# nschejtman/deepLoopCloser

Hardware: AMD Instinct MI355X
Metric: query-frames/sec vs N-keyframe DB + top-k recall@1 (higher is better)
Workload: dtype bf16; 1 GPU; 1000000 x 4096 bf16 keyframe DB, Q=256, top-20 cosine match, 1 GPU(s); db_rows=1000000, dim=4096, k=20, rows_per_gpu=1000000, pipelined=False, crowded=False

## Files before the change

### deeploopcloser_amd/_lib.py

```python
import ctypes as C
import os

_HERE = os.path.dirname(os.path.abspath(__file__))
LIB_PATH = os.path.join(_HERE, "libdlc_hip.so")

DLC_OK = 0
DLC_ERR_BAD_ARG, DLC_ERR_BAD_SHAPE, DLC_ERR_UNSUPPORTED, DLC_ERR_HIP, DLC_ERR_WORKSPACE = -1, -2, -3, -4, -5
DLC_BF16, DLC_F16, DLC_F32, DLC_F64, DLC_I8, DLC_U8 = 0, 1, 2, 3, 4, 5
DLC_ACT_NONE, DLC_ACT_SIGMOID, DLC_ACT_RELU = 0, 1, 2
DLC_B_KN, DLC_B_NK = 0, 1
DLC_MAX_K = 128
DLC_ABI_VERSION = 12
DLC_SELECT_COOP = 1
DLC_SIM_FORCE_F64, DLC_SIM_NO_HOST_SYNC = 1, 2

_vp, _i64, _int, _sz, _dbl, _flt = C.c_void_p, C.c_int64, C.c_int, C.c_size_t, C.c_double, C.c_float

SIGNATURES = {
    "dlc_abi_version": (_int, []),
    "dlc_create": (_int, [_int, C.POINTER(_vp)]),
    "dlc_destroy": (_int, [_vp]),
    "dlc_last_error": (C.c_char_p, [_vp]),
    "dlc_status_string": (C.c_char_p, [_int]),
    "dlc_gemm_bias_act": (_int, [_vp, _int, _int, _int, _i64, _i64, _i64, _vp, _i64, _vp, _i64, _vp, _vp, _i64, _vp]),
    "dlc_bias_act": (_int, [_vp, _int, _int, _i64, _i64, _vp, _i64, _vp, _vp, _i64, _vp]),
    "dlc_sdav_encode_workspace_bytes": (_sz, [_i64, C.POINTER(_i64), _int, _int]),
    "dlc_sdav_encode": (_int, [_vp, _int, _i64, _int, C.POINTER(_i64), _vp, C.POINTER(_vp), C.POINTER(_vp), _vp, _vp,
                               _sz, _vp]),
    "dlc_sdav_split_panels_bytes": (_sz, [_int, C.POINTER(_i64)]),
    "dlc_sdav_split_prepare": (_int, [_vp, _int, C.POINTER(_i64), C.POINTER(_vp), _vp, _sz, _vp]),
    "dlc_sdav_encode_split_workspace_bytes": (_sz, [_i64, C.POINTER(_i64), _int]),
    "dlc_cnnvtl_split_panels_bytes": (_sz, [_int, C.POINTER(C.c_int32)]),
    "dlc_cnnvtl_split_prepare": (_int, [_vp, _int, C.POINTER(C.c_int32), C.POINTER(_vp), _vp, _sz, _vp]),
    "dlc_cnnvtl_encode_split_workspace_bytes": (_sz, [_i64, _int, _int, _int, _int, C.POINTER(C.c_int32)]),
    "dlc_cnnvtl_encode_split": (_int, [_vp, _int, _vp, _i64, _int, _int, _int, _int, _int, C.POINTER(C.c_int32), _vp, C.POINTER(_vp),
# ... 53 lines not shown
                                    _vp, _sz, _vp]),
    "dlc_cosine_score_error_bound": (_dbl, [_i64, _i64, _i64, _int]),
    "dlc_cosine_score_error_bound_any_plan": (_dbl, [_i64]),
    "dlc_cosine_score_groups": (_int, [_vp, _int, _vp, _i64, _i64, _vp, _i64, _i64, _i64, _int, _vp, _sz, _vp]),
    "dlc_cosine_select_topk": (_int, [_vp, _int, _vp, _i64, _i64, _vp, _i64, _i64, _i64, _int, _i64, _vp, _vp, _vp, _vp, _vp, _vp,
                                     _sz, _int, _vp]),
    "dlc_cosine_groups_per_query": (_int, [_int]),
    "dlc_cosine_select_groups": (_int, [_vp, _int, _vp, _i64, _i64, _vp, _i64, _i64, _i64, _int, _vp, _sz, _vp, _vp, _int,
                                       _vp]),
    "dlc_cosine_rescore_topk": (_int, [_vp, _int, _vp, _i64, _i64, _vp, _i64, _i64, _i64, _int, _i64, _vp, _vp, _vp, _int,
                                      _vp, _vp, _vp, _vp, _int, _vp]),
    "dlc_cosine_exhaustive_topk": (_int, [_vp, _int, _vp, _i64, _i64, _vp, _i64, _i64, _i64, _int, _i64, _vp, _i64, _dbl,
                                         _vp, _vp, _vp, _vp, _vp, _vp, _sz, _vp]),
    "dlc_topk_merge_strided": (_int, [_vp, _vp, _i64, _vp, _i64, _int, _i64, _int, _vp, _dbl, _vp, _vp, _vp, _vp, _vp, _vp]),
    "dlc_topk_merge": (_int, [_vp, _vp, _vp, _int, _i64, _int, _vp, _vp, _vp, _vp]),
    "dlc_topk_keep_older": (_int, [_vp, _vp, _vp, _i64, _int, _i64, _int, _vp, _vp, _vp]),
    "dlc_cosine_scores_workspace_bytes": (_sz, [_i64, _i64, _i64]),
    "dlc_cosine_scores": (_int, [_vp, _int, _vp, _i64, _i64, _vp, _i64, _i64, _i64, _vp, _i64, _vp, _sz, _vp]),
    "dlc_host_to_device": (_int, [_vp, _vp, _vp, _sz, _vp]),
    "dlc_device_to_host": (_int, [_vp, _vp, _vp, _sz, _vp]),
    "dlc_set_host_threads": (_int, [_vp, _int]),
    "dlc_set_scratch": (_int, [_vp, _vp, _sz]),
    "dlc_set_profiling": (_int, [_vp, _int]),
    "dlc_profile_gemm_ms": (_int, [_vp, C.POINTER(_flt), _int]),
}

_lib = None


class DlcError(RuntimeError):
    """A HIP-side failure (DLC_ERR_HIP / DLC_ERR_WORKSPACE) reported by the C ABI."""


def load():
    global _lib
    if _lib is not None:
        return _lib
    if not os.path.exists(LIB_PATH):
        raise ImportError(
            "deeploopcloser_amd: %s is missing -- build it with `python -c 'import __graft_entry__ as g; g.build()'` "
            "or `make -C deeploopcloser_amd/csrc`.  There is no CPU fallback." % LIB_PATH)
    lib = C.CDLL(LIB_PATH)
    for name, (res, args) in SIGNATURES.items():
        fn = getattr(lib, name)
        fn.restype = res
        fn.argtypes = args
# ... 16 lines not shown
```

### deeploopcloser_amd/csrc/api.hip

```cpp
#include "dlc_internal.h"

#include <new>

extern "C" int dlc_abi_version(void) { return DLC_ABI_VERSION; }

extern "C" const char* dlc_status_string(int status) {
    switch (status) {
        case DLC_OK: return "ok";
        case DLC_ERR_BAD_ARG: return "bad argument";
        case DLC_ERR_BAD_SHAPE: return "bad shape";
        case DLC_ERR_UNSUPPORTED: return "unsupported dtype or mode";
        case DLC_ERR_HIP: return "HIP runtime error";
        case DLC_ERR_WORKSPACE: return "workspace too small";
        default: return "unknown status";
    }
}

extern "C" int dlc_create(int device, dlc_ctx** out) {
    if (!out) return DLC_ERR_BAD_ARG;
    *out = nullptr;
    int count = 0;
    if (hipGetDeviceCount(&count) != hipSuccess || count < 1) return DLC_ERR_HIP;
    if (device < 0 || device >= count) return DLC_ERR_BAD_ARG;
    dlc_ctx* c = new (std::nothrow) dlc_ctx;
// ... 46 lines not shown
    delete ctx->host_lock;
    delete ctx;
    return DLC_OK;
}

extern "C" const char* dlc_last_error(const dlc_ctx* ctx) { return ctx ? ctx->err : "null context"; }

extern "C" int dlc_set_scratch(dlc_ctx* ctx, void* scratch, size_t bytes) {
    if (!ctx) return DLC_ERR_BAD_ARG;
    if ((scratch && bytes == 0) || ((uintptr_t)scratch & 255))
        return dlc::fail(ctx, DLC_ERR_BAD_ARG, "set_scratch: need a 256-byte aligned buffer (or NULL, 0)");
    ctx->scratch = scratch;
    ctx->scratch_bytes = scratch ? bytes : 0;
    return DLC_OK;
}

extern "C" int dlc_set_profiling(dlc_ctx* ctx, int enabled) {
    if (!ctx) return DLC_ERR_BAD_ARG;
    ctx->profiling = enabled ? 1 : 0;
    ctx->prof_calls = 0;
    return DLC_OK;
}

extern "C" int dlc_profile_gemm_ms(dlc_ctx* ctx, float* out_ms, int capacity) {
    if (!ctx) return DLC_ERR_BAD_ARG;
    if (!out_ms || capacity < 1) return dlc::fail(ctx, DLC_ERR_BAD_ARG, "profile_gemm_ms: bad output");
    dlc::DeviceGuard guard(ctx->device);
    long long n = ctx->prof_calls;
    if (n > DLC_PROFILE_RING) n = DLC_PROFILE_RING;
    if (n > capacity) n = capacity;
    for (long long i = 0; i < n; ++i) {
        const long long call = ctx->prof_calls - n + i;
        const int slot = (int)(call % DLC_PROFILE_RING);
        DLC_HIP_CHECK(ctx, hipEventSynchronize(ctx->ev_stop[slot]));
        float ms = 0.f;
        DLC_HIP_CHECK(ctx, hipEventElapsedTime(&ms, ctx->ev_start[slot], ctx->ev_stop[slot]));
        out_ms[i] = ms;
    }
    return (int)n;
}
```

### deeploopcloser_amd/csrc/cosine_topk.hip

```cpp
#include "dlc_internal.h"

#include <algorithm>

namespace {

constexpr int BM = 256;
constexpr int BNQ = 256;
constexpr int BK = 64;
constexpr int NTHREADS = 512;
constexpr int TILE_BYTES = 256 * BK * 2;
constexpr int A_TILE = TILE_BYTES;
constexpr int B_TILE = TILE_BYTES;
#ifndef DLC_A_STAGES
#define DLC_A_STAGES 2
#endif
constexpr int A_STAGES = DLC_A_STAGES;
constexpr int B_RING = A_STAGES * A_TILE;
constexpr int LDS_BYTES = A_STAGES * A_TILE + 2 * B_TILE;
#ifndef DLC_STAGGER_SLEEP
#define DLC_STAGGER_SLEEP 15
#endif
#ifndef DLC_STAGGER_PHASES
#define DLC_STAGGER_PHASES 32
#endif
// ... 33 lines not shown
    const char* Q;
    const char* DB;
    long long ldq_b;
    long long lddb_b;
    int q;
    long long n;
    int nk;
    float* gmax;
    long long ldg;
    float* tmax;
    long long ldt;
    long long ng;
    long long nh;
    float* S;
    long long lds;
    int stagger_mult;
    int stagger_phases;
    int nqb;
    long long ntiles;
    int nsplit;
    int kchunk;
    float* P;
    long long ldp;
};

constexpr int GEMM_GROUPS = 0;
constexpr int GEMM_DENSE = 1;
constexpr int GEMM_PARTIAL = 2;

constexpr int HALF_BYTES = 128 * 128;

#ifndef DLC_A_CACHE_POLICY
#define DLC_A_CACHE_POLICY " nt"
#endif
#define DLC_DMA4_BODY(POLICY)                                \
    asm volatile(                                            \
        "s_nop 4\n\t"                                        \
        "s_mov_b32 %0, m0\n\t"                               \
        "s_mov_b32 m0, %6\n\t"                               \
        "s_nop 0\n\t"                                        \
        "global_load_lds_dwordx4 %1, %5" POLICY "\n\t"       \
        "s_add_u32 m0, %6, 0x400\n\t"                        \
        "s_nop 0\n\t"                                        \
        "global_load_lds_dwordx4 %2, %5" POLICY "\n\t"       \
        "s_add_u32 m0, %6, 0x800\n\t"                        \
        "s_nop 0\n\t"                                        \
        "global_load_lds_dwordx4 %3, %5" POLICY "\n\t"       \
// ... 186 lines not shown
        for (int c = 0; c < 4; ++c) {
            const int qidx = qblk * BNQ + wc * 64 + c * 16 + i;
            if (qidx >= p.q) continue;
#pragma unroll
            for (int t = 0; t < 8; ++t) {
                const long long row0 = tile * BM + wr * 128 + (t >> 2) * 64 + 16 * lg + 4 * (t & 3);
                *(f32x4_t*)(part + (long long)qidx * p.ldp + row0) = acc[t][c];
            }
        }
    } else if constexpr (MODE == GEMM_DENSE) {
#pragma unroll
        for (int c = 0; c < 4; ++c) {
            const int qidx = qblk * BNQ + wc * 64 + c * 16 + i;
            if (qidx >= p.q) continue;
#pragma unroll
            for (int t = 0; t < 8; ++t) {
                const long long row0 = tile * BM + wr * 128 + (t >> 2) * 64 + 16 * lg + 4 * (t & 3);
#pragma unroll
                for (int r = 0; r < 4; ++r)
                    if (row0 + r < p.n) p.S[(long long)qidx * p.lds + row0 + r] = acc[t][c][r];
            }
        }
    } else {
#pragma unroll
        for (int c = 0; c < 4; ++c) {
            const int qidx = qblk * BNQ + wc * 64 + c * 16 + i;
            float hm[2];
#pragma unroll
            for (int th = 0; th < 2; ++th) {
                float m0 = acc[th * 4][c][0], m1 = acc[th * 4 + 2][c][0];
#pragma unroll
                for (int tt = 0; tt < 2; ++tt)
#pragma unroll
                    for (int r = 0; r < 4; ++r) {
                        m0 = fmaxf(m0, acc[th * 4 + tt][c][r]);
                        m1 = fmaxf(m1, acc[th * 4 + 2 + tt][c][r]);
                    }
                hm[th] = fmaxf(m0, m1);
                const long long g = tile * (BM / GROUP) + wr * 16 + th * 8 + lg * 2;
                if (qidx < p.q) {
                    float* dst = p.gmax + (long long)qidx * p.ldg + g;
                    if (g + 1 < p.ng) *(float2*)dst = make_float2(m0, m1);
                    else if (g < p.ng) dst[0] = m0;
                }
            }
            float h = fmaxf(hm[0], hm[1]);
            h = fmaxf(h, __shfl_xor(h, 16));
            h = fmaxf(h, __shfl_xor(h, 32));
            const long long ht = tile * 2 + wr;
            if (lg == 0 && qidx < p.q && ht < p.nh) p.tmax[(long long)qidx * p.ldt + ht] = h;
        }
    }
}

template <typename Tag> struct Dot2;
template <> struct Dot2<dlc_bf16_tag> {
    typedef __attribute__((ext_vector_type(2))) __bf16 v2_t;
    static __device__ __forceinline__ float run(unsigned a, unsigned b, float c) {
        return __builtin_amdgcn_fdot2_f32_bf16(__builtin_bit_cast(v2_t, a), __builtin_bit_cast(v2_t, b), c, false);
    }
};
template <> struct Dot2<dlc_f16_tag> {
    typedef __attribute__((ext_vector_type(2))) _Float16 v2_t;
    static __device__ __forceinline__ float run(unsigned a, unsigned b, float c) {
        return __builtin_amdgcn_fdot2(__builtin_bit_cast(v2_t, a), __builtin_bit_cast(v2_t, b), c, false);
    }
};

constexpr int GEMV_MAX_Q = 4;
constexpr int GEMV_MAX_LDS = 64 * 1024;

template <typename Tag, int QB>
__global__ __launch_bounds__(256) void score_gemv_kernel(GemmArgs p) {
// ... 237 lines not shown
    float* tmax; long long ldt; int nh; int tv_in_lds;
    const float* gmax; long long ldg; long long ng;
    int kg;
    const char* Q; long long ldq_b; const char* DB; long long lddb_b;
    long long n; int d; int k; long long row_offset;
    float* out_s;
    double* out_s64;
    long long* out_i;
    int* status;
    double tau;
    const float* tau_scale;
    int* grp_ids;
    float* grp_max;
    const float* all_max;
    int parts;
    long long nq;
    int gparts;
    float* bound_out;
    const float* dense_S;
    long long ld_s;
    int rslack;
    int limited;
    long long limit0;
};
__device__ __forceinline__ long long visible_rows(long long n, int limited, long long limit0, int qi) {
    if (!limited) return n;
    const long long lim = limit0 + qi;
    return lim < 0 ? 0 : (lim < n ? lim : n);
}

template <typename Tag, int THREADS, int RS_UNROLL, int MODE>
__device__ __forceinline__ void finish_topk_body(const FinishArgs& a) {
    extern __shared__ __attribute__((aligned(16))) char dsm[];
    constexpr int FIN_WAVES = THREADS / 64;
    constexpr int FIN_THREADS = THREADS;
    constexpr int GPH = GROUPS_PER_HALF;
    const int kg = a.kg, k = a.k;
    const double tau = scaled_tau(a.tau, a.tau_scale, (int)blockIdx.x);
    const long long n = visible_rows(a.n, a.limited, a.limit0, (int)blockIdx.x);
    const long long ng = a.limited ? (n + GROUP - 1) / GROUP : a.ng;
    if (n <= 0) {
        if constexpr (MODE == FIN_GROUPS) {
            for (int e = threadIdx.x; e <= kg; e += THREADS) {
                if (e < kg) a.grp_ids[(long long)blockIdx.x * kg + e] = -1;
                a.grp_max[(long long)blockIdx.x * (kg + 1) + e] = -INFINITY;
            }
// ... 108 lines not shown
    }
    __syncthreads();
    kg2 = min(kg, m2);
    rank_select(ckey, m2, kg2, sel2, true);
    __syncthreads();
    if (sel2[kg2] >= 0) bkey = max(bkey, (unsigned)(ckey[sel2[kg2]] >> 32));
    if constexpr (MODE == FIN_GROUPS) {
        const long long W = kg + 1;
        for (int e = tid; e < kg; e += FIN_THREADS) {
            const int c = e < kg2 ? sel2[e] : -1;
            a.grp_ids[(long long)qi * kg + e] = c < 0 ? -1 : (int)key_id(ckey[c]);
            a.grp_max[(long long)qi * W + e] = c < 0 ? -INFINITY : a.gmax[(long long)qi * a.ldg + key_id(ckey[c])];
        }
        if (tid == 0) a.grp_max[(long long)qi * W + kg] = bkey ? key_f32(bkey) : -INFINITY;
        return;
    }
    if (tid < kg2) {
        const int c = sel2[tid];
        int g = c < 0 ? -1 : (int)key_id(ckey[c]);
        if (tid >= k && g >= 0 && sel2[k - 1] >= 0 && !(a.limited && !a.dense_S)) {
            const double uk = (double)key_f32((unsigned)(ckey[sel2[k - 1]] >> 32));
            if ((double)key_f32((unsigned)(ckey[c] >> 32)) < uk - 2.0 * tau) g = -2;
        }
        misc[9] = 0u;
        crow[tid] = g;
    }
    __syncthreads();
    if (tid < kg2) {
        const int g = crow[tid];
        if (g == -2) atomicMax(&misc[9], (unsigned)(ckey[sel2[tid]] >> 32));
    }
    __syncthreads();
    if (tid < kg2) sel2[tid] = crow[tid] < 0 ? -1 : crow[tid];
    bkey = max(bkey, misc[9]);
    __syncthreads();
    } else {
        kg2 = kg;
        const long long W = kg + 1;
        if (a.parts > 0) {
            unsigned bk = 0u;
            for (int e = tid; e < a.parts * (int)W; e += FIN_THREADS) {
                const int pp = e / (int)W, j = e % (int)W;
                const float v = a.all_max[((long long)pp * a.nq + qi) * W + j];
                if (v == -INFINITY) continue;
                if (j == kg) { bk = max(bk, f32_key(v)); continue; }
                int greater = 0;
                for (int p2 = 0; p2 < a.parts; ++p2) {
                    const float* av = a.all_max + ((long long)p2 * a.nq + qi) * W;
// ... 6 lines not shown
        for (int e = tid; e < kg; e += FIN_THREADS) {
            int g = a.grp_ids[(long long)qi * kg + e];
            if (g >= 0 && a.parts > 0) {
                const float v = a.grp_max[(long long)qi * W + e];
                int greater = 0;
                for (int pp = 0; pp < a.parts; ++pp) {
                    const float* av = a.all_max + ((long long)pp * a.nq + qi) * W;
                    for (int j = 0; j < kg; ++j) greater += av[j] > v ? 1 : 0;
                }
                if (greater >= kg) g = -1;
            }
            if (a.gparts > 1 && e % a.gparts != (int)blockIdx.y) g = -1;
            sel2[e] = g;
        }
        __syncthreads();
        if (a.parts > 0) bkey = misc[8];
        else {
            const float v = a.grp_max[(long long)qi * W + kg];
            bkey = v == -INFINITY ? 0u : f32_key(v);
        }
        if (a.bound_out && blockIdx.y == 0 && tid == 0) a.bound_out[qi] = bkey ? key_f32(bkey) : -INFINITY;
    }

    int m3;
    if (a.dense_S) {
        const int m = kg2 * GROUP;
        for (int e = tid; e < m; e += FIN_THREADS) {
            const int g = sel2[e / GROUP];
            const long long row = (long long)g * GROUP + (e % GROUP);
            ckey[e] = (g >= 0 && row < n) ? pack_key(a.dense_S[(long long)qi * a.ld_s + row], (unsigned)row) : 0ull;
        }
        m3 = min(k + a.rslack, m);
        for (int e = tid; e <= m3 && e < kg * GROUP; e += FIN_THREADS) crow[e] = -1;
        __syncthreads();
        if (m3 < m) rank_select(ckey, m, m3, crow, true);
        else rank_select(ckey, m, m3, crow, false);
        __syncthreads();
        if (m3 < m && crow[m3] >= 0) bkey = max(bkey, (unsigned)(ckey[crow[m3]] >> 32));
        __syncthreads();
        for (int e = tid; e < m3; e += FIN_THREADS) { const int c = crow[e]; crow[e] = c < 0 ? -1 : (int)key_id(ckey[c]); }
    } else {
        m3 = kg2 * GROUP;
        for (int e = tid; e < m3; e += FIN_THREADS) {
            const int g = sel2[e / GROUP];
            const long long row = (long long)g * GROUP + (e % GROUP);
            crow[e] = (g >= 0 && row < n) ? (int)row : -1;
        }
    }
    __syncthreads();

    const char* qrow = a.Q + (long long)qi * a.ldq_b;
    if (MODE == FIN_FUSED && a.dense_S != nullptr) {
        for (int ci = w; ci < m3; ci += FIN_WAVES) {
            const int id = __builtin_amdgcn_readfirstlane(crow[ci]);
            const double sc = id < 0 ? 0.0 : rescore1_f64<Tag>(qrow, a.DB + (long long)id * a.lddb_b, a.d, lane);
            if (lane == 0) {
                cs64[ci] = id < 0 ? -INFINITY : sc;
                ck64[ci] = id < 0 ? KEY64_EMPTY : f64_key(sc);
            }
        }
    } else
    for (int s = w; s * GROUP < m3; s += FIN_WAVES) {
        int ids[GROUP];
        bool any = false;
        const char* rows[GROUP];
#pragma unroll
        for (int r = 0; r < GROUP; ++r) {
            ids[r] = __builtin_amdgcn_readfirstlane(s * GROUP + r < m3 ? crow[s * GROUP + r] : -1);
            any |= ids[r] >= 0;
            rows[r] = a.DB + (long long)(ids[r] < 0 ? 0 : ids[r]) * a.lddb_b;
        }
        double acc[GROUP] = {0.0, 0.0, 0.0, 0.0, 0.0, 0.0, 0.0, 0.0};
        if (any) rescore8_f64<Tag, RS_UNROLL>(qrow, rows, a.d, lane, acc);
#pragma unroll
        for (int r = 0; r < GROUP; ++r)
            if (lane == r && s * GROUP + r < m3) {
                cs64[s * GROUP + r] = ids[r] < 0 ? -INFINITY : acc[r];
                ck64[s * GROUP + r] = ids[r] < 0 ? KEY64_EMPTY : f64_key(acc[r]);
            }
    }
    const long long oq = (long long)blockIdx.y * a.nq + qi;
    for (int e = tid; e < k; e += FIN_THREADS) {
        if (a.out_s) a.out_s[oq * k + e] = -INFINITY;
        a.out_s64[oq * k + e] = -INFINITY;
        a.out_i[oq * k + e] = -1;
    }
    for (int e = tid; e <= kg; e += FIN_THREADS) sel[e] = -1;
    __syncthreads();

    rank_select64(ck64, crow, m3, k, sel);
    __syncthreads();
    for (int e = tid; e < k; e += FIN_THREADS) {
        const int c = sel[e];
        if (c >= 0) {
            if (a.out_s) a.out_s[oq * k + e] = (float)cs64[c];
            a.out_s64[oq * k + e] = cs64[c];
            a.out_i[oq * k + e] = (long long)crow[c] + a.row_offset;
        }
    }
    if constexpr (MODE == FIN_FUSED) {
        if (tid == 0) {
            const int c = sel[k - 1];
// ... 552 lines not shown
    const int64_t base = dlc::cdiv(ntiles, (int64_t)8) * 8 * dlc::cdiv(q, BNQ);
    const int64_t nk = d / BK;
    SplitPlan best{1, (int)nk};
    if (base >= 256 || nk < 8) return best;
    const double t_k = 1.6, t_fix = 8.0, t_launch = 5.0, bytes_per_us = 3.0e6;
    const double part_bytes = (double)q * (double)ntiles * BM * 4.0;
    const int64_t work = ntiles * dlc::cdiv(q, BNQ);
    double best_t = (double)dlc::cdiv(work, (int64_t)256) * ((double)nk * t_k + t_fix);
    for (int64_t ns = 2; ns <= nk / 4 && ns <= 256; ++ns) {
        const int64_t kc = dlc::cdiv(nk, ns), ns_eff = dlc::cdiv(nk, kc);
        if (ns_eff != ns) continue;
        if ((double)ns_eff * part_bytes > (double)(1ll << 30)) break;
        const double t = (double)dlc::cdiv(work * ns_eff, (int64_t)256) * ((double)kc * t_k + t_fix) +
                         2.0 * (double)ns_eff * part_bytes / bytes_per_us + t_launch;
        if (t < best_t * 0.9) {
            best_t = t;
            best = SplitPlan{(int)ns_eff, (int)kc};
        }
    }
    return best;
}

struct WsLayout {
    size_t gmax, tmax, part, status, s64, rs_ids, rs_max, rs_scores, rs_idx, rs_bound, total;
    long long ldg, ldt, ldp;
    int kg;
    SplitPlan sp;
    int rparts;
    bool dense;
    double tau;
};

inline bool gemv_shape(int64_t q, int64_t nk) {
    const int qb = q <= 1 ? 1 : (q <= 2 ? 2 : 4);
    return q <= GEMV_MAX_Q && (long long)qb * nk * 128 <= GEMV_MAX_LDS;
}

constexpr int64_t DENSE_MAX_ROWS = 16384;
constexpr int DENSE_ROW_SLACK = 4;
constexpr int64_t DENSE_GEMV_BYTES = 32ll << 20;
inline bool dense_plan(int64_t q, int64_t n, int64_t d) {
    return n <= DENSE_MAX_ROWS && (!gemv_shape(q, d / BK) || n * d * 2 <= DENSE_GEMV_BYTES);
}

int rescore_parts(int64_t q, int64_t d, int kg, int k) {
    if (q > 32 || (int64_t)kg * GROUP * d * 2 < (2 << 20)) return 1;
    return std::min(kg, 2048 / k);
}

constexpr double SCORE_STEP_EPS = 1.1920928955078125e-07;
double score_error_bound(int64_t q, int64_t nk, const SplitPlan& sp, bool dense) {
    double steps;
    if (!dense && gemv_shape(q, nk)) steps = (double)nk * 0.5 + 8.0;
    else steps = 2.0 * (double)sp.kchunk + 2.0;
    return SCORE_STEP_EPS * 1.01 * steps + 3.7e-12;
}

WsLayout ws_layout(int64_t q, int64_t n, int64_t d, int k) {
    WsLayout w;
    const int64_t ntiles = dlc::cdiv(n, BM);
    w.ldg = ntiles * (BM / GROUP);
    w.ldt = ntiles * 2;
    w.kg = k + SLACK;
    size_t o = 0;
    w.gmax = o; o += dlc::align_up((size_t)q * w.ldg * 4, 256);
    w.tmax = o; o += dlc::align_up((size_t)q * w.ldt * 4, 256);
    w.sp = split_plan(q, n, d);
    w.dense = dense_plan(q, n, d);
    w.tau = score_error_bound(q, d / BK, w.sp, w.dense);
    w.ldp = ntiles * BM;
    w.part = o;
    if (w.sp.nsplit > 1 || w.dense) o += dlc::align_up((size_t)w.sp.nsplit * q * w.ldp * 4, 256);
    w.status = o; o += dlc::align_up((size_t)q * 4, 256);
    w.s64 = o; o += dlc::align_up((size_t)q * k * 8, 256);
    w.rparts = w.dense ? 1 : rescore_parts(q, d, w.kg, k);
    w.rs_ids = w.rs_max = w.rs_scores = w.rs_idx = w.rs_bound = o;
    if (w.rparts > 1) {
        w.rs_ids = o; o += dlc::align_up((size_t)q * w.kg * 4, 256);
        w.rs_max = o; o += dlc::align_up((size_t)q * (w.kg + 1) * 4, 256);
        w.rs_scores = o; o += dlc::align_up((size_t)w.rparts * q * k * 8, 256);
        w.rs_idx = o; o += dlc::align_up((size_t)w.rparts * q * k * 8, 256);
        w.rs_bound = o; o += dlc::align_up((size_t)q * 4, 256);
    }
    w.total = o;
    return w;
}

int check_operands(dlc_ctx* ctx, int dtype, const void* Q, int64_t q, int64_t ldq, const void* DB, int64_t n,
                   int64_t lddb, int64_t d) {
// ... 111 lines not shown
    WsLayout w;
};

int prepare_match(dlc_ctx* ctx, const char* what, int dtype, const void* Q, int64_t q, int64_t ldq, const void* DB,
                  int64_t n, int64_t lddb, int64_t d, int k, void* workspace, size_t workspace_bytes, MatchCall* mc) {
    int rc = check_operands(ctx, dtype, Q, q, ldq, DB, n, lddb, d);
    if (rc != DLC_OK) return rc;
    if (k < 1 || k > DLC_MAX_K) return dlc::fail(ctx, DLC_ERR_BAD_ARG, "%s: k=%d outside 1..%d", what, k, DLC_MAX_K);
    mc->w = ws_layout(q, n, d, k);
    if (!workspace || workspace_bytes < mc->w.total)
        return dlc::fail(ctx, DLC_ERR_WORKSPACE, "%s: workspace %zu < %zu bytes", what, workspace_bytes, mc->w.total);
    if (((uintptr_t)workspace & 255)) return dlc::fail(ctx, DLC_ERR_BAD_ARG, "%s: workspace must be 256-byte aligned", what);
    char* ws = (char*)workspace;
    GemmArgs& a = mc->a;
    a.Q = (const char*)Q; a.DB = (const char*)DB;
    a.ldq_b = ldq * 2; a.lddb_b = lddb * 2;
    a.q = (int)q; a.n = n; a.nk = (int)(d / BK);
    a.gmax = (float*)(ws + mc->w.gmax); a.ldg = mc->w.ldg;
    a.tmax = (float*)(ws + mc->w.tmax); a.ldt = mc->w.ldt;
    a.ng = dlc::cdiv(n, GROUP); a.nh = dlc::cdiv(n, HALF);
    a.S = nullptr; a.lds = 0;
    a.nsplit = mc->w.sp.nsplit; a.kchunk = mc->w.sp.kchunk;
    a.P = (float*)(ws + mc->w.part); a.ldp = mc->w.ldp;
    return DLC_OK;
}

inline bool small_direct(const MatchCall& mc, int k) {
    return mc.w.dense && mc.a.n <= (int64_t)FIN_THREADS * SMALL_GPT * GROUP && k + DENSE_ROW_SLACK + 1 <= SMALL_KT_MAX;
}

int run_score(dlc_ctx* ctx, int dtype, MatchCall& mc, hipStream_t st, bool partials_only = false) {
    return dlc::profiled(ctx, st, [&]() -> int {
        return (dtype == DLC_BF16) ? launch_scores<dlc_bf16_tag>(ctx, mc.a, false, st, mc.w.dense, partials_only)
                                   : launch_scores<dlc_f16_tag>(ctx, mc.a, false, st, mc.w.dense, partials_only);
    });
}

FinishArgs finish_args(const MatchCall& mc, int k, int64_t n, int64_t d, int64_t q, int64_t row_offset) {
    const GemmArgs& g = mc.a;
    FinishArgs f{};
    f.tmax = g.tmax; f.ldt = g.ldt; f.nh = (int)g.nh;
    f.gmax = g.gmax; f.ldg = g.ldg; f.ng = g.ng;
    f.kg = mc.w.kg;
    f.Q = g.Q; f.ldq_b = g.ldq_b; f.DB = g.DB; f.lddb_b = g.lddb_b;
    f.n = n; f.d = (int)d; f.k = k; f.row_offset = row_offset;
    f.tau = mc.w.tau;
    f.nq = q;
    return f;
}

template <typename Tag, int THREADS, int RS_UNROLL, int MODE>
int launch_finish(dlc_ctx* ctx, FinishArgs f, int64_t q, bool small_lds, hipStream_t st) {
    size_t dsm = fin_lds_fixed(f.kg);
    f.tv_in_lds = MODE != FIN_RESCORE && !small_lds && (size_t)f.nh * 4 <= 96 * 1024;
    if (f.tv_in_lds) dsm += (size_t)f.nh * 4;
    dsm = dlc::align_up(dsm, 16);
    void (*fk)(FinishArgs);
    if constexpr (THREADS == 256) fk = finish_topk_coop_kernel<Tag, RS_UNROLL, MODE>;
    else fk = finish_topk_kernel<Tag, THREADS, RS_UNROLL, MODE>;
    if (dsm > 48 * 1024)
        DLC_HIP_CHECK(ctx, hipFuncSetAttribute((const void*)fk, hipFuncAttributeMaxDynamicSharedMemorySize, (int)dsm));
    hipLaunchKernelGGL(fk, dim3((unsigned)q, (unsigned)(MODE == FIN_RESCORE && f.gparts > 1 ? f.gparts : 1)), dim3(THREADS),
                       dsm, st, f);
    DLC_LAUNCH_CHECK(ctx, "finish_topk_kernel");
    return DLC_OK;
}

template <int MODE>
int run_select(dlc_ctx* ctx, int dtype, const FinishArgs& f, int64_t q, int flags, hipStream_t st) {
    const bool coop = (flags & DLC_SELECT_COOP) != 0;
// ... 21 lines not shown
    DLC_LAUNCH_CHECK(ctx, "exhaustive_topk_kernel");
    return DLC_OK;
}

int launch_merge(dlc_ctx* ctx, const double* scores, int64_t score_part_stride, const int64_t* idx, int64_t idx_part_stride,
                 int parts, int64_t q, int k, const float* bound, double tau, const float* tau_scale, float* out_scores,
                 double* out_scores_f64, int64_t* out_idx, int* status, hipStream_t st) {
    const size_t m = (size_t)parts * k;
    const size_t dsm = m * 24;
    if (dsm > 48 * 1024) return dlc::fail(ctx, DLC_ERR_BAD_SHAPE, "topk_merge: parts*k=%zu too large (max 2048)", m);
    hipLaunchKernelGGL(merge_topk_kernel, dim3((unsigned)q), dim3(FIN_THREADS), dsm, st, scores, (long long)score_part_stride,
                       (const long long*)idx, (long long)idx_part_stride, parts, (long long)q, k, bound, tau, tau_scale,
                       out_scores, out_scores_f64, (long long*)out_idx, status);
    DLC_LAUNCH_CHECK(ctx, "merge_topk_kernel");
    return DLC_OK;
}

int run_finish(dlc_ctx* ctx, int dtype, const MatchCall& mc, int k, int64_t n, int64_t d, int64_t q, int64_t row_offset,
               float* out_scores, double* out_scores_f64, int64_t* out_idx, int32_t* out_status, void* workspace, int flags,
               const float* tau_scale, hipStream_t st, int limited = 0, int64_t limit0 = 0, bool direct = false) {
    char* ws = (char*)workspace;
    FinishArgs f = finish_args(mc, k, n, d, q, row_offset);
    f.limited = limited; f.limit0 = limit0; f.tau_scale = tau_scale;
    int* status = out_status ? out_status : (int*)(ws + mc.w.status);
    double* s64 = out_scores_f64 ? out_scores_f64 : (double*)(ws + mc.w.s64);
    int rc;
    if (direct) {
        SmallArgs sa{};
        sa.P = mc.a.P; sa.ldp = mc.a.ldp; sa.qstride = (long long)q * mc.a.ldp; sa.nsplit = mc.a.nsplit;
        sa.gmax = mc.a.gmax; sa.ldg = mc.a.ldg;
        sa.Q = f.Q; sa.ldq_b = f.ldq_b; sa.DB = f.DB; sa.lddb_b = f.lddb_b;
        sa.n = n; sa.d = (int)d; sa.k = k; sa.m3max = k + DENSE_ROW_SLACK; sa.row_offset = row_offset;
        sa.out_s = out_scores; sa.out_s64 = s64; sa.out_i = (long long*)out_idx; sa.status = status; sa.tau = mc.w.tau;
        sa.tau_scale = tau_scale; sa.limited = limited; sa.limit0 = limit0;
        const bool long_rows = d >= 16384;
        if (dtype == DLC_BF16) {
            if (long_rows) hipLaunchKernelGGL(small_topk_long_kernel<dlc_bf16_tag>, dim3((unsigned)q), dim3(FIN_THREADS), 0, st, sa);
            else hipLaunchKernelGGL(small_topk_kernel<dlc_bf16_tag>, dim3((unsigned)q), dim3(FIN_THREADS), 0, st, sa);
        } else {
            if (long_rows) hipLaunchKernelGGL(small_topk_long_kernel<dlc_f16_tag>, dim3((unsigned)q), dim3(FIN_THREADS), 0, st, sa);
            else hipLaunchKernelGGL(small_topk_kernel<dlc_f16_tag>, dim3((unsigned)q), dim3(FIN_THREADS), 0, st, sa);
        }
        DLC_LAUNCH_CHECK(ctx, "small_topk_kernel");
    } else if (mc.w.rparts <= 1) {
        f.out_s = out_scores; f.out_s64 = s64; f.out_i = (long long*)out_idx; f.status = status;
        if (mc.w.dense) { f.dense_S = mc.a.P; f.ld_s = mc.a.ldp; f.rslack = DENSE_ROW_SLACK; }
// ... 397 lines not shown
```

### deeploopcloser_amd/csrc/dlc_internal.h

```cpp
#pragma once
#include <hip/hip_runtime.h>
#include <stdint.h>
#include <stdarg.h>
#include <stdio.h>
#include <string.h>
#include <mutex>

#include "../../include/dlc.h"

struct dlc_host_staging;

struct dlc_ctx {
    int device;
    char err[512];
    int profiling;
    long long prof_calls;
    hipEvent_t ev_start[DLC_PROFILE_RING];
    hipEvent_t ev_stop[DLC_PROFILE_RING];
    void* scratch;
    size_t scratch_bytes;
    unsigned long long func_attr_set;
    void* zero_page;
    dlc_host_staging* staging;
    std::mutex* host_lock;
    int host_threads;
    unsigned long long* host_flag;
    hipEvent_t ev_flag;
};

enum {
    DLC_ATTR_GEMM_BASE = 0,
    DLC_ATTR_GEMV_BASE = 16,
    DLC_ATTR_DGEMM_BASE = 24,
    DLC_ATTR_DMA64_BASE = 32,
    DLC_ATTR_PAIR_TILE = 48,
    DLC_ATTR_GRAM_I8 = 49,
    DLC_ATTR_PAIR_FILTER = 50,
    DLC_ATTR_SPLIT_F16 = 51,
    DLC_ATTR_DS_DMA = 52,
    DLC_ATTR_CONV_SPLIT_F16 = 53,
};

namespace dlc {

void staging_free(dlc_host_staging* s);

inline int fail(dlc_ctx* ctx, int status, const char* fmt, ...) {
    if (ctx) {
        va_list ap;
        va_start(ap, fmt);
// ... 75 lines not shown
```

### deeploopcloser_amd/engine.py

```python
import collections
import contextlib
import ctypes as C
import weakref

import numpy as np
import torch

from . import _lib as L

_TORCH_TO_DLC = {torch.bfloat16: L.DLC_BF16, torch.float16: L.DLC_F16, torch.float32: L.DLC_F32,
                 torch.float64: L.DLC_F64, torch.int8: L.DLC_I8}
_NAME_TO_TORCH = {"bf16": torch.bfloat16, "bfloat16": torch.bfloat16, "f16": torch.float16, "fp16": torch.float16,
                  "float16": torch.float16, "f32": torch.float32, "float32": torch.float32, "f64": torch.float64,
                  "float64": torch.float64}

SCRATCH_BYTES = 256 << 20
K_STEP = 64


TopK = collections.namedtuple("TopK", "scores idx scores_f64 status")


_RAW_STREAM = getattr(torch._C, "_cuda_getCurrentRawStream", None)

# ... 992 lines not shown
        if out is None:
            o_s = torch.empty((nq, k), dtype=torch.float32, device=self.device)
            o_i = torch.empty((nq, k), dtype=torch.int64, device=self.device)
        else:
            o_s = self._check_out("out[0] (scores)", out[0], (nq, k), torch.float32)
            o_i = self._check_out("out[1] (idx)", out[1], (nq, k), torch.int64)
        o_64 = torch.empty((nq, k), dtype=torch.float64, device=self.device) if details else None
        self._check(self.lib.dlc_topk_merge(self.ctx, _ptr(scores_f64), _ptr(idx), parts, nq, k, _ptr(o_s), _ptr(o_64),
                                             _ptr(o_i), self._stream()))
        return TopK(o_s, o_i, o_64, None) if details else (o_s, o_i)

    def cosine_scores(self, q, db):
        self._check_stored(q, db)
        nq, d = q.shape
        n = db.shape[0]
        s = torch.empty((nq, n), dtype=torch.float32, device=self.device)
        need = self.lib.dlc_cosine_scores_workspace_bytes(nq, n, d)
        ws = self.workspace("scores", need) if need else None
        self._check(self.lib.dlc_cosine_scores(self.ctx, _TORCH_TO_DLC[q.dtype], _ptr(q), nq, q.stride(0), _ptr(db), n,
                                                db.stride(0), d, _ptr(s), s.stride(0), _ptr(ws) if need else None,
                                                need, self._stream()))
        return s

    def set_profiling(self, enabled):
        self._check(self.lib.dlc_set_profiling(self.ctx, 1 if enabled else 0))

    def profile_gemm_ms(self, capacity=256):
        buf = (C.c_float * capacity)()
        n = self.lib.dlc_profile_gemm_ms(self.ctx, buf, capacity)
        if n < 0:
            self._check(n)
        return [float(buf[i]) for i in range(n)]


_default = {}


def default_engine(device=None):
    if device is None:
        if not torch.cuda.is_available():
            L.load()
            raise RuntimeError("deeploopcloser_amd needs a visible MI355X; there is no CPU fallback")
        device = torch.cuda.current_device()
    elif not isinstance(device, int):
        device = torch.device(device).index or 0
    if device not in _default:
# ... 3 lines not shown
```

### include/dlc.h

```cpp
#ifndef DLC_H_
#define DLC_H_

#include <stddef.h>
#include <stdint.h>

#ifdef __cplusplus
extern "C" {
#endif

#define DLC_ABI_VERSION 12

typedef struct dlc_ctx dlc_ctx;

typedef enum dlc_status {
    DLC_OK = 0,
    DLC_ERR_BAD_ARG = -1,
    DLC_ERR_BAD_SHAPE = -2,
    DLC_ERR_UNSUPPORTED = -3,
    DLC_ERR_HIP = -4,
    DLC_ERR_WORKSPACE = -5
} dlc_status;

typedef enum dlc_dtype {
    DLC_BF16 = 0,
    DLC_F16 = 1,
    DLC_F32 = 2,
    DLC_F64 = 3,
    DLC_I8 = 4,
    DLC_U8 = 5
} dlc_dtype;

typedef enum dlc_act {
    DLC_ACT_NONE = 0,
// ... 121 lines not shown
int dlc_sdav_stream_query_batch(dlc_ctx* ctx, void* state, size_t state_bytes, int64_t capacity, int64_t P, int64_t H,
                                const double* desc, int64_t f_first, int64_t n_queries, const double* score, double a,
                                double b, double* rows_out, int64_t ld_rows, int64_t* stats, void* workspace,
                                size_t workspace_bytes, void* stream);
int dlc_sdav_stream_query_batch_staged(dlc_ctx* ctx, void* state, size_t state_bytes, int64_t capacity, int64_t P, int64_t H,
                                       const double* desc, int64_t f_first, int64_t n_queries, const double* score, double a,
                                       double b, double* rows_out, int64_t ld_rows, int64_t* stats, void* workspace,
                                       size_t workspace_bytes, int stage, void* stream);
int dlc_topk_rows_f64(dlc_ctx* ctx, const double* scores, int64_t rows, int64_t ld, int64_t limit0, int64_t limit_step,
                      int k, double* out_scores, int64_t* out_idx, const int64_t* poison, void* stream);
int dlc_cnnvtl_distance_matrix(dlc_ctx* ctx, const int8_t* desc, int64_t N, int64_t D, int64_t ldd,
                               int64_t* out, void* stream);
size_t dlc_cnnvtl_distance_topk_workspace_bytes(int64_t Q, int64_t N, int64_t D, int k);
int dlc_cnnvtl_distance_topk(dlc_ctx* ctx, const int8_t* queries, int64_t Q, int64_t ldq,
                             const int8_t* db, int64_t N, int64_t ldd, int64_t D,
                             int64_t limit0, int64_t limit_step, int k,
                             int64_t* out_dist, int64_t* out_idx,
                             void* workspace, size_t workspace_bytes, void* stream);

int dlc_l2_normalize_rows(dlc_ctx* ctx, int src_dtype, const void* src, int64_t n, int64_t d, int64_t lds,
                          int center, int dst_dtype, void* dst, int64_t ldd, void* stream);
#define DLC_MAX_K 128
size_t dlc_cosine_topk_workspace_bytes(int64_t q, int64_t n, int64_t d, int k);
int dlc_cosine_topk(dlc_ctx* ctx, int dtype, const void* Q, int64_t q, int64_t ldq,
                    const void* DB, int64_t n, int64_t lddb, int64_t d, int k, int64_t row_offset,
                    float* out_scores, double* out_scores_f64, int64_t* out_idx, int32_t* out_status,
                    const float* tau_scale, void* workspace, size_t workspace_bytes, void* stream);
int dlc_max_row_norm(dlc_ctx* ctx, int dtype, const void* rows, int64_t n, int64_t ld, int64_t d, float* max_norm,
                     void* stream);
int dlc_cosine_tau_scale(dlc_ctx* ctx, int dtype, const void* Q, int64_t q, int64_t ldq, int64_t d,
                         const float* db_max_norm, float* tau_scale, void* stream);
int dlc_cosine_topk_older(dlc_ctx* ctx, int dtype, const void* Q, int64_t q, int64_t ldq,
                          const void* DB, int64_t n, int64_t lddb, int64_t d, int k, int64_t row_offset, int64_t limit0,
                          float* out_scores, double* out_scores_f64, int64_t* out_idx, int32_t* out_status,
                          const float* tau_scale, void* workspace, size_t workspace_bytes, void* stream);
double dlc_cosine_score_error_bound(int64_t q, int64_t n, int64_t d, int k);
double dlc_cosine_score_error_bound_any_plan(int64_t d);
#define DLC_SELECT_COOP 1
int dlc_cosine_score_groups(dlc_ctx* ctx, int dtype, const void* Q, int64_t q, int64_t ldq,
                            const void* DB, int64_t n, int64_t lddb, int64_t d, int k,
                            void* workspace, size_t workspace_bytes, void* stream);
int dlc_cosine_select_topk(dlc_ctx* ctx, int dtype, const void* Q, int64_t q, int64_t ldq,
                           const void* DB, int64_t n, int64_t lddb, int64_t d, int k, int64_t row_offset,
                           float* out_scores, double* out_scores_f64, int64_t* out_idx, int32_t* out_status,
                           const float* tau_scale, void* workspace, size_t workspace_bytes, int flags, void* stream);
int dlc_cosine_groups_per_query(int k);
// ... 44 lines not shown
```

Before: 126,800 query-frames/s.

## Record per-group argmax hints to rescore single rows instead of whole groups

The group-max GEMM epilogue now also records, per 8-row group, the argmax row and a coarse exponent code for the gap between the max and second-largest value, stored as a byte in a new workspace buffer. The finish/rescore kernel reads these hints, and when the gap is large enough that no other row in the group can reach the top-k threshold, it rescores only the argmax row, processed three at a time per wave, instead of all eight rows. This is meant to cut f64 rescore DB reads and compute, at the cost of extra syncthreads and shared-memory staging in the GEMM epilogue plus more workspace. Hints are used only for non-dense, non-GEMV, unsplit-K plans without row limits, and can be turned off through a new context flag.

Result: slower. 125,300 query-frames/s (-1.1%).

```diff
diff --git a/deeploopcloser_amd/_lib.py b/deeploopcloser_amd/_lib.py
--- a/deeploopcloser_amd/_lib.py
+++ b/deeploopcloser_amd/_lib.py
@@ -10,7 +10,7 @@
 DLC_ACT_NONE, DLC_ACT_SIGMOID, DLC_ACT_RELU = 0, 1, 2
 DLC_B_KN, DLC_B_NK = 0, 1
 DLC_MAX_K = 128
-DLC_ABI_VERSION = 12
+DLC_ABI_VERSION = 13
 DLC_SELECT_COOP = 1
 DLC_SIM_FORCE_F64, DLC_SIM_NO_HOST_SYNC = 1, 2
 
@@ -110,6 +110,7 @@
     "dlc_set_host_threads": (_int, [_vp, _int]),
     "dlc_set_scratch": (_int, [_vp, _vp, _sz]),
     "dlc_set_profiling": (_int, [_vp, _int]),
+    "dlc_set_topk_row_hints": (_int, [_vp, _int]),
     "dlc_profile_gemm_ms": (_int, [_vp, C.POINTER(_flt), _int]),
 }
 
diff --git a/deeploopcloser_amd/csrc/api.hip b/deeploopcloser_amd/csrc/api.hip
--- a/deeploopcloser_amd/csrc/api.hip
+++ b/deeploopcloser_amd/csrc/api.hip
@@ -92,6 +92,12 @@
     return DLC_OK;
 }
 
+extern "C" int dlc_set_topk_row_hints(dlc_ctx* ctx, int enabled) {
+    if (!ctx) return DLC_ERR_BAD_ARG;
+    ctx->no_row_hints = enabled ? 0 : 1;
+    return DLC_OK;
+}
+
 extern "C" int dlc_profile_gemm_ms(dlc_ctx* ctx, float* out_ms, int capacity) {
     if (!ctx) return DLC_ERR_BAD_ARG;
     if (!out_ms || capacity < 1) return dlc::fail(ctx, DLC_ERR_BAD_ARG, "profile_gemm_ms: bad output");
diff --git a/deeploopcloser_amd/csrc/cosine_topk.hip b/deeploopcloser_amd/csrc/cosine_topk.hip
--- a/deeploopcloser_amd/csrc/cosine_topk.hip
+++ b/deeploopcloser_amd/csrc/cosine_topk.hip
@@ -79,7 +79,24 @@
     int kchunk;
     float* P;
     long long ldp;
+    unsigned char* hint;
 };
+
+constexpr int HINT_MIN_EXP = -15;
+constexpr int HINT_MAX_CODE = 17;
+__device__ __forceinline__ unsigned hint_byte(float m, float second, int arg) {
+    const float dgap = m - second;
+    int c = 0;
+    if (dgap > 0.0f) {
+        c = (int)((__float_as_uint(dgap) - 1u) >> 23) - 127 - HINT_MIN_EXP + 1;
+        c = c < 0 ? 0 : (c > HINT_MAX_CODE ? HINT_MAX_CODE : c);
+    }
+    return ((unsigned)c << 3) | (unsigned)arg;
+}
+__host__ __device__ inline int hint_slot(int gi) { return (gi & 17) | (((gi >> 1) & 3) << 2) | (((gi >> 3) & 1) << 1); }
+__host__ __device__ inline double hint_gap(unsigned code) {
+    return (double)(1u << code) * (1.0 / 65536.0);
+}
 
 constexpr int GEMM_GROUPS = 0;
 constexpr int GEMM_DENSE = 1;
@@ -312,20 +329,30 @@
             }
         }
     } else {
+        if (p.hint) __syncthreads();
 #pragma unroll
         for (int c = 0; c < 4; ++c) {
             const int qidx = qblk * BNQ + wc * 64 + c * 16 + i;
             float hm[2];
+            unsigned hw = 0u;
 #pragma unroll
             for (int th = 0; th < 2; ++th) {
-                float m0 = acc[th * 4][c][0], m1 = acc[th * 4 + 2][c][0];
-#pragma unroll
-                for (int tt = 0; tt < 2; ++tt)
-#pragma unroll
-                    for (int r = 0; r < 4; ++r) {
-                        m0 = fmaxf(m0, acc[th * 4 + tt][c][r]);
-                        m1 = fmaxf(m1, acc[th * 4 + 2 + tt][c][r]);
+                float gm[2];
+#pragma unroll
+                for (int gs = 0; gs < 2; ++gs) {
+                    float mx = acc[th * 4 + gs * 2][c][0], second = -INFINITY;
+                    int arg = 0;
+#pragma unroll
+                    for (int e = 1; e < GROUP; ++e) {
+                        const float v = acc[th * 4 + gs * 2 + (e >> 2)][c][e & 3];
+                        second = __builtin_amdgcn_fmed3f(mx, second, v);
+                        arg = v > mx ? e : arg;
+                        mx = fmaxf(mx, v);
                     }
+                    gm[gs] = mx;
+                    hw |= hint_byte(mx, second, arg) << (8 * (th * 2 + gs));
+                }
+                const float m0 = gm[0], m1 = gm[1];
                 hm[th] = fmaxf(m0, m1);
                 const long long g = tile * (BM / GROUP) + wr * 16 + th * 8 + lg * 2;
                 if (qidx < p.q) {
@@ -334,11 +361,18 @@
                     else if (g < p.ng) dst[0] = m0;
                 }
             }
+            if (p.hint) ((unsigned*)smem)[(wc * 64 + c * 16 + i) * 8 + wr * 4 + lg] = hw;
             float h = fmaxf(hm[0], hm[1]);
             h = fmaxf(h, __shfl_xor(h, 16));
             h = fmaxf(h, __shfl_xor(h, 32));
             const long long ht = tile * 2 + wr;
             if (lg == 0 && qidx < p.q && ht < p.nh) p.tmax[(long long)qidx * p.ldt + ht] = h;
+        }
+        if (p.hint) {
+            __syncthreads();
+            const int ql = tid >> 1;
+            if (qblk * BNQ + ql < p.q)
+                *(uint4*)(p.hint + ((tile * p.q + (long long)qblk * BNQ) << 5) + tid * 16) = ((const uint4*)smem)[tid];
         }
     }
 }
@@ -622,6 +656,7 @@
     int rslack;
     int limited;
     long long limit0;
+    const unsigned char* hint;
 };
 __device__ __forceinline__ long long visible_rows(long long n, int limited, long long limit0, int qi) {
     if (!limited) return n;
@@ -776,8 +811,17 @@
             const double uk = (double)key_f32((unsigned)(ckey[sel2[k - 1]] >> 32));
             if ((double)key_f32((unsigned)(ckey[c] >> 32)) < uk - 2.0 * tau) g = -2;
         }
+        int one = -1;
+        if (a.hint && g >= 0 && sel2[k - 1] >= 0 && !a.limited) {
+            const unsigned h = a.hint[(((long long)(g >> 5) * a.nq + qi) << 5) + hint_slot(g & 31)];
+            const double uk = (double)key_f32((unsigned)(ckey[sel2[k - 1]] >> 32));
+            const long long row = (long long)g * GROUP + (h & 7u);
+            if ((h >> 3) && row < n && (double)key_f32((unsigned)(ckey[c] >> 32)) - hint_gap(h >> 3) < uk - 2.0 * tau)
+                one = (int)row;
+        }
         misc[9] = 0u;
         crow[tid] = g;
+        sel[tid] = one;
     }
     __syncthreads();
     if (tid < kg2) {
@@ -830,7 +874,7 @@
         if (a.bound_out && blockIdx.y == 0 && tid == 0) a.bound_out[qi] = bkey ? key_f32(bkey) : -INFINITY;
     }
 
-    int m3;
+    int m3, ns = 0, nf = 0;
     if (a.dense_S) {
         const int m = kg2 * GROUP;
         for (int e = tid; e < m; e += FIN_THREADS) {
@@ -848,11 +892,21 @@
         __syncthreads();
         for (int e = tid; e < m3; e += FIN_THREADS) { const int c = crow[e]; crow[e] = c < 0 ? -1 : (int)key_id(ckey[c]); }
     } else {
-        m3 = kg2 * GROUP;
-        for (int e = tid; e < m3; e += FIN_THREADS) {
-            const int g = sel2[e / GROUP];
-            const long long row = (long long)g * GROUP + (e % GROUP);
-            crow[e] = (g >= 0 && row < n) ? (int)row : -1;
+        int my = 0;
+        for (int j = 0; j < kg2; ++j) {
+            const bool kept = sel2[j] >= 0, single = kept && sel[j] >= 0;
+            if (j == tid) my = single ? ns : nf;
+            ns += single ? 1 : 0;
+            nf += (kept && !single) ? 1 : 0;
+        }
+        m3 = ns + nf * GROUP;
+        if (tid < kg2 && sel2[tid] >= 0) {
+            if (sel[tid] >= 0) crow[my] = sel[tid];
+            else
+                for (int r = 0; r < GROUP; ++r) {
+                    const long long row = (long long)sel2[tid] * GROUP + r;
+                    crow[ns + my * GROUP + r] = row < n ? (int)row : -1;
+                }
         }
     }
     __syncthreads();
@@ -867,14 +921,39 @@
                 ck64[ci] = id < 0 ? KEY64_EMPTY : f64_key(sc);
             }
         }
-    } else
-    for (int s = w; s * GROUP < m3; s += FIN_WAVES) {
+    } else {
+    const int ntrip = (ns + 2) / 3;
+    for (int s = w; s < ntrip + nf; s += FIN_WAVES) {
+        if (s < ntrip) {
+            const int c0 = s * 3, cnt = min(3, ns - c0);
+            const char* rows[3];
+#pragma unroll
+            for (int r = 0; r < 3; ++r)
+                rows[r] = a.DB + (long long)__builtin_amdgcn_readfirstlane(crow[c0 + (r < cnt ? r : 0)]) * a.lddb_b;
+            double acc[3] = {0.0, 0.0, 0.0};
+            constexpr int U1 = RS_UNROLL >= 4 ? 4 : 2;
+            if (cnt == 3) rescore_rows_f64<Tag, 3, U1>(qrow, rows, a.d, lane, acc);
+            else if (cnt == 2) {
+                const char* const r2[2] = {rows[0], rows[1]};
+                double a2[2];
+                rescore_rows_f64<Tag, 2, U1>(qrow, r2, a.d, lane, a2);
+                acc[0] = a2[0]; acc[1] = a2[1];
+            } else acc[0] = rescore1_f64<Tag>(qrow, rows[0], a.d, lane);
+#pragma unroll
+            for (int r = 0; r < 3; ++r)
+                if (lane == r && r < cnt) {
+                    cs64[c0 + r] = acc[r];
+                    ck64[c0 + r] = f64_key(acc[r]);
+                }
+            continue;
+        }
+        const int c0 = ns + (s - ntrip) * GROUP;
         int ids[GROUP];
         bool any = false;
         const char* rows[GROUP];
 #pragma unroll
         for (int r = 0; r < GROUP; ++r) {
-            ids[r] = __builtin_amdgcn_readfirstlane(s * GROUP + r < m3 ? crow[s * GROUP + r] : -1);
+            ids[r] = __builtin_amdgcn_readfirstlane(crow[c0 + r]);
             any |= ids[r] >= 0;
             rows[r] = a.DB + (long long)(ids[r] < 0 ? 0 : ids[r]) * a.lddb_b;
         }
@@ -882,10 +961,11 @@
         if (any) rescore8_f64<Tag, RS_UNROLL>(qrow, rows, a.d, lane, acc);
 #pragma unroll
         for (int r = 0; r < GROUP; ++r)
-            if (lane == r && s * GROUP + r < m3) {
-                cs64[s * GROUP + r] = ids[r] < 0 ? -INFINITY : acc[r];
-                ck64[s * GROUP + r] = ids[r] < 0 ? KEY64_EMPTY : f64_key(acc[r]);
-            }
+            if (lane == r) {
+                cs64[c0 + r] = ids[r] < 0 ? -INFINITY : acc[r];
+                ck64[c0 + r] = ids[r] < 0 ? KEY64_EMPTY : f64_key(acc[r]);
+            }
+    }
     }
     const long long oq = (long long)blockIdx.y * a.nq + qi;
     for (int e = tid; e < k; e += FIN_THREADS) {
@@ -1484,7 +1564,7 @@
 }
 
 struct WsLayout {
-    size_t gmax, tmax, part, status, s64, rs_ids, rs_max, rs_scores, rs_idx, rs_bound, total;
+    size_t gmax, tmax, hint, part, status, s64, rs_ids, rs_max, rs_scores, rs_idx, rs_bound, total;
     long long ldg, ldt, ldp;
     int kg;
     SplitPlan sp;
@@ -1527,6 +1607,7 @@
     size_t o = 0;
     w.gmax = o; o += dlc::align_up((size_t)q * w.ldg * 4, 256);
     w.tmax = o; o += dlc::align_up((size_t)q * w.ldt * 4, 256);
+    w.hint = o; o += dlc::align_up((size_t)q * w.ldg, 256);
     w.sp = split_plan(q, n, d);
     w.dense = dense_plan(q, n, d);
     w.tau = score_error_bound(q, d / BK, w.sp, w.dense);
@@ -1684,6 +1765,7 @@
     a.S = nullptr; a.lds = 0;
     a.nsplit = mc->w.sp.nsplit; a.kchunk = mc->w.sp.kchunk;
     a.P = (float*)(ws + mc->w.part); a.ldp = mc->w.ldp;
+    a.hint = (unsigned char*)(ws + mc->w.hint);
     return DLC_OK;
 }
 
@@ -1708,6 +1790,7 @@
     f.n = n; f.d = (int)d; f.k = k; f.row_offset = row_offset;
     f.tau = mc.w.tau;
     f.nq = q;
+    f.hint = (!mc.w.dense && !use_gemv(g) && g.nsplit <= 1) ? g.hint : nullptr;
     return f;
 }
 
@@ -1775,6 +1858,7 @@
     char* ws = (char*)workspace;
     FinishArgs f = finish_args(mc, k, n, d, q, row_offset);
     f.limited = limited; f.limit0 = limit0; f.tau_scale = tau_scale;
+    if (ctx->no_row_hints) f.hint = nullptr;
     int* status = out_status ? out_status : (int*)(ws + mc.w.status);
     double* s64 = out_scores_f64 ? out_scores_f64 : (double*)(ws + mc.w.s64);
     int rc;
diff --git a/deeploopcloser_amd/csrc/dlc_internal.h b/deeploopcloser_amd/csrc/dlc_internal.h
--- a/deeploopcloser_amd/csrc/dlc_internal.h
+++ b/deeploopcloser_amd/csrc/dlc_internal.h
@@ -26,6 +26,7 @@
     int host_threads;
     unsigned long long* host_flag;
     hipEvent_t ev_flag;
+    int no_row_hints;
 };
 
 enum {
diff --git a/deeploopcloser_amd/engine.py b/deeploopcloser_amd/engine.py
--- a/deeploopcloser_amd/engine.py
+++ b/deeploopcloser_amd/engine.py
@@ -1038,6 +1038,9 @@
                                                 need, self._stream()))
         return s
 
+    def set_topk_row_hints(self, enabled):
+        self._check(self.lib.dlc_set_topk_row_hints(self.ctx, 1 if enabled else 0))
+
     def set_profiling(self, enabled):
         self._check(self.lib.dlc_set_profiling(self.ctx, 1 if enabled else 0))
 
diff --git a/include/dlc.h b/include/dlc.h
--- a/include/dlc.h
+++ b/include/dlc.h
@@ -8,7 +8,7 @@
 extern "C" {
 #endif
 
-#define DLC_ABI_VERSION 12
+#define DLC_ABI_VERSION 13
 
 typedef struct dlc_ctx dlc_ctx;
 
@@ -176,6 +176,7 @@
                           int center, int dst_dtype, void* dst, int64_t ldd, void* stream);
 #define DLC_MAX_K 128
 size_t dlc_cosine_topk_workspace_bytes(int64_t q, int64_t n, int64_t d, int k);
+int dlc_set_topk_row_hints(dlc_ctx* ctx, int enabled);
 int dlc_cosine_topk(dlc_ctx* ctx, int dtype, const void* Q, int64_t q, int64_t ldq,
                     const void* DB, int64_t n, int64_t lddb, int64_t d, int k, int64_t row_offset,
                     float* out_scores, double* out_scores_f64, int64_t* out_idx, int32_t* out_status,
```
